# foobaz/pngloss

Hardware: AMD Instinct MI355X
Metric: Mpixels/s (filter+quantise path), 4096x4096 RGBA8 s=19; bit-exact vs ref (higher is better)
Workload: dtype u8

## Files before the change

### pngloss_amd/csrc/pl_seg_core.h

```cpp
#ifndef PL_SEG_CORE_H
#define PL_SEG_CORE_H

#include <stdint.h>
#include <stddef.h>
#include <string.h>

#include "pl_result.h"

#if defined(__HIPCC__)
#define PLS_HD __host__ __device__ __forceinline__
#else
#define PLS_HD inline
#endif

#if defined(__HIP_DEVICE_COMPILE__)
#define PLS_THREADS(tid, nt) for (int tid = (int)threadIdx.x, pls_once_ = 1; pls_once_ && tid < (int)(nt); pls_once_ = 0)
#define PLS_SYNC() __syncthreads()
#define PLS_ATOMIC_ADD(p, v) atomicAdd((p), (v))
#define PLS_ATOMIC_MIN(p, v) atomicMin((p), (v))
#define PLS_ATOMIC_OR(p, v) atomicOr((p), (v))
#define PLS_ATOMIC_CAS(p, cmp, v) atomicCAS((p), (cmp), (v))
#define PLS_ATOMIC_ADD_RET(p, v) atomicAdd((p), (v))
#define PLS_ATOMIC_EXCH(p, v) atomicExch((p), (v))
#define PLS_ATOMIC_ADD64(p, v) atomicAdd((unsigned long long *)(p), (unsigned long long)(v))
#define PLS_CLOCK() wall_clock64()
#define PLS_ATOMIC_MAX(p, v) atomicMax((p), (v))
#define PLS_WAVE_LEADER(tid) (((tid) & 63) == 0)
__device__ __forceinline__ uint32_t pls_wave_sum_u32(uint32_t v) { for (int o = 32; o > 0; o >>= 1) v += __shfl_xor(v, o, 64); return v; }
__device__ __forceinline__ uint64_t pls_wave_sum_u64(uint64_t v) { for (int o = 32; o > 0; o >>= 1) v += __shfl_xor(v, o, 64); return v; }
__device__ __forceinline__ int pls_wave_max_i(int v) { for (int o = 32; o > 0; o >>= 1) { const int t = __shfl_xor(v, o, 64); v = t > v ? t : v; } return v; }
__device__ __forceinline__ int pls_wave_min_i(int v) { for (int o = 32; o > 0; o >>= 1) { const int t = __shfl_xor(v, o, 64); v = t < v ? t : v; } return v; }
#define PLS_ATOMIC_MAX_I(p, v) atomicMax((p), (v))
#define PLS_ATOMIC_MAX_U(p, v) atomicMax((p), (v))
#define PLS_ATOMIC_MIN_I(p, v) atomicMin((p), (v))
#define PLS_HOST_VISIBLE_ADD(p, v) __hip_atomic_fetch_add((p), (v), __ATOMIC_RELAXED, __HIP_MEMORY_SCOPE_SYSTEM)
#define PLS_HOST_VISIBLE_STORE(p, v) __hip_atomic_store((p), (v), __ATOMIC_RELAXED, __HIP_MEMORY_SCOPE_SYSTEM)
#else
#define PLS_THREADS(tid, nt) for (int tid = 0; tid < (int)(nt); ++tid)
#define PLS_SYNC() ((void)0)
#define PLS_ATOMIC_ADD(p, v) (*(p) += (v))
#define PLS_ATOMIC_MIN(p, v) (*(p) = *(p) < (v) ? *(p) : (v))
#define PLS_ATOMIC_OR(p, v) (*(p) |= (v))
inline uint32_t pls_host_cas(uint32_t *p, uint32_t cmp, uint32_t v) { const uint32_t old = *p; if (old == cmp) *p = v; return old; }
inline uint32_t pls_host_add_ret(uint32_t *p, uint32_t v) { const uint32_t old = *p; *p += v; return old; }
#define PLS_ATOMIC_CAS(p, cmp, v) pls_host_cas((p), (cmp), (v))
#define PLS_ATOMIC_ADD_RET(p, v) pls_host_add_ret((p), (v))
#define PLS_ATOMIC_EXCH(p, v) (*(p) = (v))
#define PLS_ATOMIC_ADD64(p, v) (*(p) += (v))
#define PLS_CLOCK() 0ull
#define PLS_ATOMIC_MAX(p, v) (*(p) = *(p) > (v) ? *(p) : (v))
#define PLS_WAVE_LEADER(tid) (true)
inline uint32_t pls_wave_sum_u32(uint32_t v) { return v; }
inline uint64_t pls_wave_sum_u64(uint64_t v) { return v; }
inline int pls_wave_max_i(int v) { return v; }
inline int pls_wave_min_i(int v) { return v; }
#define PLS_ATOMIC_MAX_I(p, v) (*(p) = *(p) > (v) ? *(p) : (v))
#define PLS_ATOMIC_MAX_U(p, v) (*(p) = *(p) > (v) ? *(p) : (v))
#define PLS_ATOMIC_MIN_I(p, v) (*(p) = *(p) < (v) ? *(p) : (v))
#define PLS_HOST_VISIBLE_ADD(p, v) (*(p) += (v))
#define PLS_HOST_VISIBLE_STORE(p, v) (*(p) = (v))
#endif

#if defined(__HIP_DEVICE_COMPILE__) && !defined(SEG_PLAIN_POINTERS)
#define SEG_AS_LDS __attribute__((address_space(3)))
#define SEG_AS_GLB __attribute__((address_space(1)))
#else
#define SEG_AS_LDS
#define SEG_AS_GLB
#endif
typedef SEG_AS_LDS uint32_t *seg_lds_u32;
typedef SEG_AS_LDS uint8_t *seg_lds_u8;
typedef SEG_AS_LDS uint16_t *seg_lds_u16;

#if defined(__HIPCC__)
#define PLS_UNROLL _Pragma("unroll")
#else
#define PLS_UNROLL
#endif
#define SEG_NFILT 5
#ifndef SEG_DEBUG_ROW
#define SEG_DEBUG_ROW(kind, failed, winner, start_none)
#endif
#ifndef SEG_DEBUG_REPAIR
#define SEG_DEBUG_REPAIR(f, c, sg, est, sid)
#endif
#ifndef SEG_DEBUG_BREAK
#define SEG_DEBUG_BREAK(f, c, sg, est, y)
#endif
#ifndef SEG_DEBUG_STATE
#define SEG_DEBUG_STATE(f, k, sl, i, ps)
#endif
#ifndef SEG_DEBUG_COUNT
#define SEG_DEBUG_COUNT(slot, v)
#endif
#ifndef SEG_L
#define SEG_L 32
#endif
#ifndef SEG_UNIT
#define SEG_UNIT 3
#endif
#define SEG_UNIT_MIN_SEGS 680
#define SEG_SEEDS1_MIN_SEGS 330
#define SEG_SEEDS1_MIN_SEGS_PER_IMAGE 32
#define SEG_UNIT_MIN_SEGS_SEEDS 1000
#if !defined(SEG_UNC) && SEG_UNIT > 6
#define SEG_UNC 7
#endif
#ifndef SEG_UNC
#define SEG_UNC 10
#endif
#ifndef SEG_UNC_SEEDS
#define SEG_UNC_SEEDS 16
#endif
#ifndef SEG_UNC_SEEDS1
#define SEG_UNC_SEEDS1 8
#endif
#define SEG_UNC_SEEDS_OF(unit) ((unit) == 1 ? SEG_UNC_SEEDS1 : SEG_UNC_SEEDS)
#ifndef SEG_UNT
#define SEG_UNT 512
#endif
#define SEG_UPOOL SEG_UNT
#define SEG_GRP 16
#define SEG_VGRP 8
#define SEG_VGRP_UNITS 16
#ifndef SEG_TPARTS_BATCH
#define SEG_TPARTS_BATCH 1
#endif
#define SEG_VGRP_OF(tparts) ((tparts) == SEG_TPARTS_BATCH ? SEG_VGRP_UNITS : SEG_VGRP)
#define SEG_TPARTS 4
#define SEG_COMMIT_W 256
#define SEG_CTL_IMG_OF(P) (SEG_NFILT * (P).tparts)
#define SEG_PARTS 4
#define SEG_PL (SEG_L / SEG_PARTS)
#define SEG_NSP 256
#define SEG_NS_MAX 1024
#define SEG_TOFF 384
#define SEG_TN 768
#define SEG_TBL_WORDS (4 * SEG_TN + 128)
#define SEG_INVALID 0xFFFFu
#define SEG_NOFAIL 0xFFFFFFFFu
#define SEG_MAGIC 0x5E6C0DE1u
#define SEG_MAX_RESTARTS 12
#define SEG_NG_BURST 16
#define SEG_MAX_WIDTH (1u << 20)
#define SEG_THREADS 1024
#define SEG_CHAIN_THREADS 1024
#define SEG_CHAIN_THREADS_UNIT 256
#define SEG_REPLAY_THREADS (SEG_GRP * SEG_L)
#define SEG_REPLAY_NT_BATCH SEG_REPLAY_THREADS
#define SEG_REPLAY_NT (2 * SEG_REPLAY_THREADS)
#define SEG_KEYLUT_MAX 8192
#define SEG_NSS 32
#define SEG_SMALL_SEGS 8
#define SEG_ENUM_NT_SMALL_MAX_NSEG 320
#define SEG_KEYS_MAX 2048
#ifndef SEG_KA_SEEDED
#define SEG_KA_SEEDED 4
#endif
#define SEG_KIN 32
#define SEG_SEED_LANES 64
#define SEG_SEED_LONG_AFTER 2u
#define SEG_SEED_KMAX 16
#define SEG_EH 512
#define SEG_EHW 8
#define SEG_EH_WORDS (SEG_EH + SEG_EHW - 4)
#define SEG_EH_EMPTY 0xFFFFFFFFu

enum { SEG_K_INIT = 0, SEG_K_RESTART, SEG_K_RETRY, SEG_K_COMMIT, SEG_K_ABORT, SEG_K_FINISHED };

struct SegParams {
    int32_t strength, bleed;
    int32_t ns;
    int32_t dmax, cmax, tmax;
// ... 866 lines not shown
            }
            keys[tid] = key;
        }
        PLS_SYNC();
        PLS_THREADS(tid, NT) {
            if ((uint32_t)tid < DA0 + DA1) {
                const int c = (uint32_t)tid < DA0 ? 0 : 1;
                const uint32_t i = c ? (uint32_t)tid - DA0 : (uint32_t)tid;
                const uint32_t key = keys[tid];
                if (key != SEG_NOKEY && (i == 0 || keys[tid - 1] != key)) {
                    const uint32_t base = seg_eh_base(key);
                    for (int q = 0; q < SEG_EHW; q++) {
                        const uint32_t old = PLS_ATOMIC_CAS(&ht[c * SEG_EH_WORDS + base + q], SEG_NOKEY, key);
                        if (old == SEG_NOKEY) {
                            const uint32_t d = PLS_ATOMIC_ADD_RET(&trflag[SEG_TF_NDISTINCT + c], 1u);
                            dense[c * SEG_EH_WORDS + base + q] = (uint16_t)(d < SEG_NSP ? d : 0xffffu);
                            if (d < SEG_NSP) uniq[c * SEG_NSP + d] = key;
                            break;
                        }
                        if (old == key) break;
                    }
                }
            }
        }
        PLS_SYNC();
    } else {
    PLS_THREADS(tid, NT) {
        const int c = tid / SEG_NSP, i = tid % SEG_NSP;
        const uint32_t key = keys[tid];
        if (key != SEG_NOKEY && (i == 0 || keys[tid - 1] != key)) {
            const uint32_t base = seg_eh_base(key);
            for (int q = 0; q < SEG_EHW; q++) {
                const uint32_t old = PLS_ATOMIC_CAS(&ht[c * SEG_EH_WORDS + base + q], SEG_NOKEY, key);
                if (old == SEG_NOKEY) {
                    const uint32_t d = PLS_ATOMIC_ADD_RET(&trflag[SEG_TF_NDISTINCT + c], 1u);
                    dense[c * SEG_EH_WORDS + base + q] = (uint16_t)(d < SEG_NSP ? d : 0xffffu);
                    if (d < SEG_NSP) uniq[c * SEG_NSP + d] = key;
                    break;
                }
                if (old == key) break;
            }
        }
    }
    PLS_SYNC();
    }
    if (prof) te[2] = PLS_CLOCK();
    PLS_THREADS(tid, NT) {
        for (int i = tid; i < NCH * SEG_EH_WORDS; i += NT) {
            const int lc = i / SEG_EH_WORDS;
            if ((uint32_t)(c0 + lc) >= bpp) continue;
            const uint32_t k = ht[i], d = dense[i];
            j.ehash[(((size_t)f * j.nseg + seg) * 4 + c0) * SEG_EH_WORDS + i] = (k == SEG_NOKEY || d >= SEG_NSP) ? SEG_EH_EMPTY : ((k << 8) | d);
        }
    }
    PLS_THREADS(tid, NT) {
        uint32_t Dc[NCH];
        for (int k = 0; k < NCH; k++) Dc[k] = trflag[SEG_TF_NDISTINCT + k] < SEG_NSP ? trflag[SEG_TF_NDISTINCT + k] : SEG_NSP;
        int lc = 0, i = tid;
        uint32_t D = Dc[0];
        PLS_UNROLL
        for (int k = 0; k + 1 < NCH; k++) if (lc == k && (uint32_t)i >= Dc[k]) { i -= (int)Dc[k]; lc = k + 1; D = Dc[k + 1]; }
        const int c = c0 + lc;
        if (tid < NCH && (uint32_t)(c0 + tid) < bpp) j.dcnt[((size_t)f * j.nseg + seg) * 4 + c0 + tid] = trflag[SEG_TF_NDISTINCT + tid] < SEG_NSP ? trflag[SEG_TF_NDISTINCT + tid] : SEG_NSP;
        if ((uint32_t)c < bpp && (uint32_t)i < D) {
            SegState st = seg_eh_state(uniq[lc * SEG_NSP + i]);
            const size_t slot = (((size_t)f * j.nseg + seg) * 4 + c) * SEG_NSP + i;
            const SegPix *ps = px + (nrun + 1) * 4 + c;
            int bad = 0;
            for (int part = 0; part < SEG_PARTS; part++) {
                if (part) j.rck[slot * (SEG_PARTS - 1) + (part - 1)] = bad ? 0xFFFFFFFFu : seg_state_pack(st);
                bad |= seg_run_fast_f(f, trx, ps + part * SEG_PL * 4, 4, SEG_PL, st, SEG_LDS_CU32(tw), G, SEG_LDS_CU32(lut));
            }
            j.rst[slot] = bad ? 0xFFFFFFFFu : seg_state_pack(st);
        }
        if (prof && tid == 0) {
            te[3] = PLS_CLOCK(); te[4] = te[3];
            for (int q = 0; q < PLR_SEG_ENUM_PHASES; q++) { PLS_ATOMIC_MAX(&j.result[PLR_SEG_ENUM_MAX + q], (int32_t)(te[q + 1] - te[q])); PLS_ATOMIC_ADD((uint32_t *)&j.result[PLR_SEG_ENUM_SUM + q], (uint32_t)(te[q + 1] - te[q])); }
            PLS_ATOMIC_ADD((uint32_t *)&j.result[PLR_SEG_ENUM_RUNS], 1u);
            PLS_ATOMIC_ADD((uint32_t *)&j.result[PLR_SEG_ENUM_STATES], two_stage ? 2u * (trflag[SEG_TF_NDISTINCT] + trflag[SEG_TF_NDISTINCT + 1]) : trflag[SEG_TF_NDISTINCT] + trflag[SEG_TF_NDISTINCT + 1] + trflag[SEG_TF_NDISTINCT + 2] + trflag[SEG_TF_NDISTINCT + 3]);
        }
    }
}

template <int NT>
PLS_HD void seg_enum_small_body(const SegJob &j, const SegParams &P, const SegCtlView &cv, int par, int f, int seg0, unsigned char *smem)
{
    if (cv.finished || cv.active != 1) return;
    const uint32_t W = j.W, bpp = j.bpp;
    constexpr int NSEGS = NT / (4 * SEG_NSS);
    if ((uint32_t)(seg0 + NSEGS) * SEG_L <= cv.start_x) return;
    typedef SegLdsSmall<NT> LDS;
    uint32_t *tw = LDS::tw(smem), *lut = LDS::lut(smem);
    SegPix *px = LDS::px(smem);
    const uint32_t y = cv.y;
    const uint32_t *row = seg_row_orig(j, y), *nab = y ? j.img + (size_t)(y - 1u) * W : nullptr, *e0g = seg_e0(j, y);
    const SegGeo G = seg_geo((int)cv.s);
    uint32_t *trflag = LDS::trflag(smem);
    PLS_THREADS(tid, NT) { if (tid == 0) *trflag = 0u; }
    PLS_SYNC();
    PLS_THREADS(tid, NT) {
        constexpr int NTW = (SEG_TBL_WORDS + NT - 1) / NT;
        uint32_t vt[NTW], vl = 0;
        SegPixRaw vp = seg_pix_raw_zero();
        PLS_UNROLL
        for (int q = 0; q < NTW; q++) { const int i = tid + q * NT; vt[q] = i < SEG_TBL_WORDS ? j.tables[(size_t)f * SEG_TBL_WORDS + i] : 0u; }
        if (tid < 512) vl = P.lut_a[tid];
        if (tid < NSEGS * SEG_L) vp = seg_pix_fetch(row, nab, e0g, (uint32_t)seg0 * SEG_L + (uint32_t)tid, W);
        PLS_UNROLL
        for (int q = 0; q < NTW; q++) { const int i = tid + q * NT; if (i < SEG_TBL_WORDS) tw[i] = vt[q]; }
        if (tid < 512) lut[tid] = vl;
        if (tid < NSEGS * SEG_L) {
            seg_pix_split4(px + tid * 4, vp, bpp, (uint32_t)seg0 * SEG_L + (uint32_t)tid, W);
            if ((bpp & 1u) == 0u && (px[tid * 4 + (bpp - 1u)].w >> 24)) PLS_ATOMIC_OR(trflag, 1u);
        }
    }
    PLS_SYNC();
    const bool trx = *trflag != 0u;
    PLS_THREADS(tid, NT) {
        const int sl = tid / (4 * SEG_NSS), c = (tid / SEG_NSS) & 3, i = tid % SEG_NSS;
        const uint32_t seg = (uint32_t)seg0 + (uint32_t)sl, x0 = seg * SEG_L;
        if (seg < j.nseg && x0 < W && (x0 > cv.start_x || cv.start_x == 0) && (uint32_t)c < bpp && i < P.ns_small) {
            SegState st;
            uint32_t out = SEG_INVALID;
            const size_t slot = (((size_t)f * j.nseg + seg) * 4 + c) * SEG_NSP + i;
            if (seg_small_decode(P, i, st)) {
                int bad = 0;
                for (int part = 0; part < SEG_PARTS; part++) {
                    if (part) j.rck[slot * (SEG_PARTS - 1) + (part - 1)] = bad ? 0xFFFFFFFFu : seg_state_pack(st);
                    bad |= seg_run_fast_f<SEG_PL>(f, trx, px + (sl * SEG_L + part * SEG_PL) * 4 + c, 4, st, SEG_LDS_CU32(tw), G, SEG_LDS_CU32(lut));
                }
                if (!bad) out = seg_small_encode(P, st);
            } else {
                for (int part = 1; part < SEG_PARTS; part++) j.rck[slot * (SEG_PARTS - 1) + (part - 1)] = 0xFFFFFFFFu;
            }
            j.maps[(((size_t)f * j.nseg + seg) * 4 + c) * (size_t)P.nsp + i] = (uint16_t)i;
            j.rout[(((size_t)f * j.nseg + seg) * 4 + c) * SEG_NSP + i] = (uint16_t)out;
            j.rst[(((size_t)f * j.nseg + seg) * 4 + c) * SEG_NSP + i] = out == SEG_INVALID ? 0xFFFFFFFFu : seg_state_pack(st);
            if (i == 0) j.dcnt[((size_t)f * j.nseg + seg) * 4 + c] = (uint32_t)P.ns_small;
        }
    }
}

PLS_HD uint32_t seg_bits_count(const uint32_t *bits, uint32_t a, uint32_t b)
{
    uint32_t n = 0;
    for (uint32_t w = a >> 5; w <= (b ? (b - 1u) >> 5 : 0u) && a < b; w++) {
        uint32_t m = bits[w];
        if (w == (a >> 5)) m &= 0xFFFFFFFFu << (a & 31u);
        if (w == ((b - 1u) >> 5) && (b & 31u)) m &= 0xFFFFFFFFu >> (32u - (b & 31u));
        n += (uint32_t)__builtin_popcount(m);
    }
    return n;
}
template <int LANES, int UNIT, int NC, bool SEEDS = false>
PLS_HD void seg_enum_unit_body(const SegJob &j, const SegParams &P, const SegCtlView &cv, int par, int f, int grp, unsigned char *smem)
{
    if (cv.finished || cv.active != 1) return;
    constexpr int NT = SEG_UNT, HT = 2 * LANES;
    constexpr int CPR = NT / LANES < NC ? NT / LANES : NC;
    constexpr int ROUNDS = (NC + CPR - 1) / CPR;
    constexpr uint32_t E = UNIT, UL = E * SEG_L, NPX = UL + 1;
    static_assert(CPR * HT <= 2 * SEG_UNT && CPR * LANES <= SEG_UNT && NC <= 24 && NC * (UNIT * SEG_L + 1) <= SEG_UNPX, "hash tables, per-turn lists, pixel records and the bookkeeping words are sized for this");
    const uint32_t W = j.W, bpp = j.bpp, nseg = j.nseg, nunit = (nseg + E - 1) / E, ncombo = nunit * bpp;
    const uint32_t q0 = (uint32_t)grp * NC;
    if (q0 >= ncombo) return;
    const uint32_t sx = cv.start_x;
    { const uint32_t ql = seg_umin(q0 + NC, ncombo) - 1u; if (sx && (ql / bpp) * UL <= sx) return; }
    constexpr uint32_t NP1 = SEEDS ? SEG_SEED_KMAX + 1 : SEG_UN_K1MAX + 1;
    typedef SegLdsUnit<LANES, UNIT, NC, SEEDS> LDS;
    uint32_t *tw = LDS::tw(smem), *lut = LDS::lut(smem), *pool = LDS::pool(smem), *misc = LDS::misc(smem);
    uint32_t *ht = LDS::ht(smem), *uniqr = LDS::uniqr(smem), *keys = LDS::keys(smem);
    uint16_t *dense = LDS::dense(smem), *mapl = LDS::mapl(smem);
    SegPix *px1 = SEEDS ? LDS::px1_seeds(smem) : LDS::px1_std(smem);
    static_assert(!SEEDS || LANES == SEG_SEED_LANES, "one lane per seed");
    const int KR = SEEDS ? seg_min(seg_max(j.nbreak >= SEG_SEED_LONG_AFTER ? P.seed_kin + P.seed_kin / 2 : P.seed_kin, 1), SEG_SEED_KMAX) : 0;
    SegPix *px = LDS::px(smem);
    uint32_t *pool2 = LDS::pool2(smem);
    static_assert(SEG_K1 <= SEG_UN_K1MAX && SEG_K1_ONE_CHUNK <= SEG_UN_K1MAX, "the first phase's records");
    const uint32_t y = cv.y;
    const SEG_AS_GLB uint32_t *row = seg_row_orig(j, y), *nab = y ? j.img + (size_t)(y - 1u) * W : nullptr, *e0g = seg_e0(j, y);
    const SegGeo G = seg_geo((int)cv.s);
    const int nstates = seg_is_small(P, f) ? P.ns_small : P.ns;
    const bool prof = (P.engine_flags & 1) != 0 && LANES == SEG_NSP;
    unsigned long long te[5] = { 0, 0, 0, 0, 0 };
    if (prof) te[0] = PLS_CLOCK();
    PLS_THREADS(tid, NT) { if (tid < 128) misc[tid] = 0u; }
    PLS_SYNC();
    PLS_THREADS(tid, NT) {
        constexpr int NTW = (SEG_TBL_WORDS + NT - 1) / NT;
        static_assert(NC * (SEG_UN_K1MAX + 1) <= NT, "one first-phase record per thread");
        uint32_t vt[NTW], vl = 0;
        SegPix vp = seg_pix_make(0, 0, 0, 0, 0);
        PLS_UNROLL
        for (int q = 0; q < NTW; q++) { const int i = tid + q * NT; vt[q] = i < SEG_TBL_WORDS ? j.tables[(size_t)f * SEG_TBL_WORDS + i] : 0u; }
        if (tid < 512) vl = P.lut_a[tid];
        {
            const uint32_t k = (uint32_t)tid / NP1, pq = (uint32_t)tid % NP1, cq = q0 + k;
            if (k < (uint32_t)NC && cq < ncombo) {
                const uint32_t u = cq / bpp, c = cq % bpp, x = SEEDS ? u * UL + pq - 1u - (uint32_t)KR : u * UL + pq - 1u;
                if (x < W && (!SEEDS || pq <= (uint32_t)KR)) vp = seg_pix_load(row, nab, e0g, bpp, x, (int)c);
            }
        }
        PLS_UNROLL
        for (int q = 0; q < NTW; q++) { const int i = tid + q * NT; if (i < SEG_TBL_WORDS) tw[i] = vt[q]; }
        if (tid < 512) lut[tid] = vl;
        if ((uint32_t)tid < (uint32_t)NC * NP1) { px1[tid] = vp; if (vp.w >> 24) PLS_ATOMIC_OR(&misc[SEG_UM_TRANSPARENT], 1u); }
    }
    PLS_SYNC();
    const bool trx1 = misc[SEG_UM_TRANSPARENT] != 0u;
    if (prof) te[1] = PLS_CLOCK();
    const int K1 = SEEDS ? 0 : seg_k1(nstates);
    for (int r = 0; r < ROUNDS; r++) {
        PLS_THREADS(tid, NT) {
            for (int i = tid; i < CPR * HT; i += NT) ht[i] = 0xffffffffu;
            if (tid < CPR) misc[SEG_UM_TURN_N + tid] = 0u;
            if (SEEDS) for (int i = tid; i < CPR * 128; i += NT) ((uint32_t *)mapl)[i] = 0xffffffffu;
        }
        PLS_SYNC();
        if (SEEDS) {
            PLS_THREADS(tid, NT) {
                const int kk = tid / LANES, k = r * CPR + kk, i = tid % LANES;
// ... 1935 lines not shown
```

### pngloss_amd/csrc/pl_seg_lds.h

```cpp
#ifndef PL_SEG_LDS_H
#define PL_SEG_LDS_H

#ifndef PL_SEG_CORE_H
#error "pl_seg_lds.h is a part of pl_seg_core.h: include that"
#endif

#define SEG_HT 512
#ifndef SEG_UNC_SMALL
#define SEG_UNC_SMALL (SEG_UNIT <= 3 ? 20 : (SEG_UNIT <= 4 ? 15 : (SEG_UNIT <= 6 ? 10 : 7)))
#endif
#define SEG_UNC_SMALL_OF(unit) ((unit) == SEG_UNIT ? SEG_UNC_SMALL : (SEG_UNC_SMALL < 20 ? SEG_UNC_SMALL : 20))
#define SEG_UNPX (SEG_UNC_SMALL * (SEG_UNIT * SEG_L + 1))
#define SEG_UN_K1MAX 4
#define SEG_CBLK 16
#define SEG_CR_SH 6
#define SEG_CR_MAX (1 << SEG_CR_SH)
#define SEG_CHAIN_CAP 256
#define SEG_CHAIN_CAP8 224
#define SEG_CHAIN_POS (SEG_CHAIN_CAP + 32)
#define SEG_CHAIN_TROWS(n) (((n) < SEG_CHAIN_CAP8 ? (n) : SEG_CHAIN_CAP8) + SEG_CBLK + 2)
#define SEG_CHAIN_TBYTES(n) ((size_t)SEG_CHAIN_TROWS(n) * 512)
#define SEG_CHAIN_GWORDS ((SEG_CHAIN_CAP / SEG_CBLK + 2) * 256 / 2)
#ifndef SEG_WATCH_OF
#define SEG_WATCH_OF(V) ((V) > 8 ? 2 : 8)
// ... 44 lines not shown
    int first, last;
    const char *when;
};
struct SegLdsPlaced { uint32_t off[SEG_LDS_MAX_ROWS], bytes[SEG_LDS_MAX_ROWS], end; bool sound; };
constexpr SegLdsPlaced seg_lds_place(const SegLdsRegion *t, int n)
{
    SegLdsPlaced p = {};
    uint32_t rel[SEG_LDS_MAX_ROWS] = {};
    int first[SEG_LDS_MAX_ROWS] = {}, last[SEG_LDS_MAX_ROWS] = {};
    for (int k = 0; k < n; k++) {
        first[k] = t[k].kind == 2 ? first[k - 1] : t[k].first; last[k] = t[k].kind == 2 ? last[k - 1] : t[k].last;
        p.bytes[k] = t[k].count == SEG_LDS_FITS ? 0u : t[k].elem_bytes * t[k].count;
        rel[k] = t[k].kind == 2 ? rel[k - 1] + p.bytes[k - 1] : 0u;
    }
    for (int k = 0; k < n; k++)
        if (t[k].count == SEG_LDS_FITS)
            for (int q = 0; q < n; q++) if (t[q].kind && first[q] == k && last[q] == k && rel[q] + p.bytes[q] > p.bytes[k]) p.bytes[k] = rel[q] + p.bytes[q];
    for (int k = 0; k < n; k++) if (!t[k].kind) { p.off[k] = p.end; p.end += p.bytes[k]; }
    p.sound = n <= SEG_LDS_MAX_ROWS;
    for (int k = 0; k < n; k++) {
        if (t[k].kind) { p.off[k] = p.off[first[k]] + rel[k]; if (p.off[k] + p.bytes[k] > p.off[last[k]] + p.bytes[last[k]]) p.sound = false; }
        if (p.off[k] % t[k].align) p.sound = false;
    }
    return p;
}
constexpr uint32_t seg_lds_max(uint32_t a) { return a; }
template <class... R> constexpr uint32_t seg_lds_max(uint32_t a, R... r) { return a > seg_lds_max(r...) ? a : seg_lds_max(r...); }

#define SEG_LDS_ID_R(name, T, AS, n) i_##name,
#define SEG_LDS_ID_O(name, T, AS, n, first, last, when) i_##name,
#define SEG_LDS_ROW_R(name, T, AS, n) SegLdsRegion{ #name, 0u, (uint32_t)sizeof(T), (uint32_t)(n), (uint32_t)sizeof(T), 0, -1, -1, nullptr },
#define SEG_LDS_ROW_O(name, T, AS, n, first, last, when) SegLdsRegion{ #name, 0u, (uint32_t)sizeof(T), (uint32_t)(n), (uint32_t)sizeof(T), 1, i_##first, i_##last, when },
#define SEG_LDS_ROW_B(name, T, AS, n) SegLdsRegion{ #name, 0u, (uint32_t)sizeof(T), (uint32_t)(n), (uint32_t)sizeof(T), 2, -1, -1, nullptr },
#define SEG_LDS_GET_R(name, T, AS, n) static PLS_HD AS T *name(unsigned char *smem) { constexpr uint32_t o = Table::placed(0).off[Table::i_##name]; return (AS T *)((AS unsigned char *)smem + o); }
#define SEG_LDS_GET_O(name, T, AS, n, first, last, when) SEG_LDS_GET_R(name, T, AS, n)
#define SEG_LDS_VAR_BYTES(n) ((uint32_t)SEG_CHAIN_TBYTES(n))
#define SEG_LDS_GET_V(name, T, AS, n) static PLS_HD AS T *name(unsigned char *smem, uint32_t npos) { \
        constexpr uint32_t o = Table::placed(0).off[Table::i_##name] - SEG_LDS_VAR_BYTES(0); \
        static_assert(o + SEG_LDS_VAR_BYTES(60) == Table::placed(60).off[Table::i_##name] && o + SEG_LDS_VAR_BYTES(SEG_CHAIN_CAP + 1) == Table::placed(SEG_CHAIN_CAP + 1).off[Table::i_##name], "the table's offset"); \
        return (AS T *)((AS unsigned char *)smem + o + SEG_LDS_VAR_BYTES(npos)); }
#define SEG_LDS_ALIGN_X(name, bytes) if (i == i_##name) t.align = (bytes);
#define SEG_LDS_UNPAREN(...) __VA_ARGS__
#define SEG_LDS_LAYOUT(Name, LIST, ALIGN, HEAD, ARGS) \
    SEG_LDS_UNPAREN HEAD struct Name##Table { \
        enum { LIST(SEG_LDS_ID_R, SEG_LDS_ID_O, SEG_LDS_ID_R, SEG_LDS_ID_R) n_regions }; \
        static constexpr SegLdsRegion row(int i, uint32_t n) { (void)n; const SegLdsRegion all[] = { LIST(SEG_LDS_ROW_R, SEG_LDS_ROW_O, SEG_LDS_ROW_B, SEG_LDS_ROW_R) }; SegLdsRegion t = all[i]; ALIGN(SEG_LDS_ALIGN_X) return t; } \
        static constexpr SegLdsPlaced placed(uint32_t n) { SegLdsRegion t[n_regions] = {}; for (int i = 0; i < n_regions; i++) t[i] = row(i, n); return seg_lds_place(t, n_regions); } \
        static constexpr SegLdsRegion region(int i, uint32_t n = 0) { SegLdsRegion r = row(i, n); const SegLdsPlaced p = placed(n); r.offset = p.off[i]; if (r.count == SEG_LDS_FITS) r.count = p.bytes[i] / r.elem_bytes; return r; } \
        static constexpr uint32_t end(uint32_t n = 0) { return placed(n).end; } \
    }; \
    SEG_LDS_UNPAREN HEAD struct Name { \
        typedef Name##Table SEG_LDS_UNPAREN ARGS Table; \
        static_assert(Table::placed(1).sound && Table::placed(SEG_CHAIN_CAP + 1).sound, #Name ": every region starts on a multiple of its alignment, every overlay lies inside its place"); \
        LIST(SEG_LDS_GET_R, SEG_LDS_GET_O, SEG_LDS_GET_R, SEG_LDS_GET_V) \
    };

#define SEG_LDS_ALIGN_NONE(X)


#define SEG_LDS_ENUM(R, O, B, V) \
    R(tw, uint32_t, , SEG_TBL_WORDS)                   \
    R(px, SegPix, , (SEG_L + 1) * 4)                   \
    R(lut, uint32_t, , 512)                            \
    R(trflag, uint32_t, , 8)                           \
    R(ht, uint32_t, , 4 * SEG_HT)                      \
    R(dense, uint16_t, , 4 * SEG_HT)                   \
    R(uniq, uint32_t, , 4 * SEG_NSP)                   \
    R(res, uint16_t, , 4 * SEG_NSP)                    \
    R(lslot, uint16_t, , NT)                           \
    R(keys, uint32_t, , NT)
SEG_LDS_LAYOUT(SegLdsEnum, SEG_LDS_ENUM, SEG_LDS_ALIGN_NONE, (template <int NT>), (<NT>))

#define SEG_LDS_SEEDED(R, O, B, V) \
    R(tw, uint32_t, , SEG_TBL_WORDS) \
    R(px, SegPix, , (SEG_KIN + SEG_L + 1) * 4)         \
    R(lut, uint32_t, , 512) \
    R(trflag, uint32_t, , 8)                           \
    R(ht, uint32_t, , 4 * SEG_EH_WORDS)                \
    R(dense, uint16_t, , 4 * SEG_EH_WORDS)             \
    R(uniq, uint32_t, , 4 * SEG_NSP)                   \
    R(keys, uint32_t, , NT)
SEG_LDS_LAYOUT(SegLdsSeeded, SEG_LDS_SEEDED, SEG_LDS_ALIGN_NONE, (template <int NT>), (<NT>))

#define SEG_LDS_SMALL(R, O, B, V) \
    R(tw, uint32_t, , SEG_TBL_WORDS) \
    R(lut, uint32_t, , 512) \
    R(px, SegPix, , NT / (4 * SEG_NSS) * SEG_L * 4)    \
    R(trflag, uint32_t, , 1)
SEG_LDS_LAYOUT(SegLdsSmall, SEG_LDS_SMALL, SEG_LDS_ALIGN_NONE, (template <int NT>), (<NT>))

#define SEG_LDS_UNIT_CPR (SEG_UNT / LANES < NC ? SEG_UNT / LANES : NC)
#define SEG_LDS_UNIT(R, O, B, V) \
    R(tw, uint32_t, , SEG_TBL_WORDS) \
    R(lut, uint32_t, , 512) \
    R(pool, uint32_t, , SEG_UPOOL)                     \
    R(px1_std, SegPix, , SEG_UNC_SMALL * (SEG_UN_K1MAX + 1))    \
    R(misc, uint32_t, , 128)                           \
    R(work, unsigned char, , SEG_LDS_FITS) \
    O(ht, uint32_t, , 2 * SEG_UNT, work, work, "in the first phase")    \
    B(dense, uint16_t, , 2 * SEG_UNT)                  \
    B(uniqr, uint32_t, , SEG_UNT)                      \
    B(keys, uint32_t, , SEG_UNT)                       \
    B(px1_seeds, SegPix, , SEEDS ? NC * (SEG_SEED_KMAX + 1) : 0)    \
    B(mapl, uint16_t, , SEEDS ? SEG_LDS_UNIT_CPR * 256 : 0)      \
    O(px, SegPix, , SEG_UNPX, work, work, "in the second phase, behind the barrier that ends the first")    \
    B(pool2, uint32_t, , SEG_UPOOL)
SEG_LDS_LAYOUT(SegLdsUnit, SEG_LDS_UNIT, SEG_LDS_ALIGN_NONE, (template <int LANES, int UNIT, int NC, bool SEEDS>), (<LANES, UNIT, NC, SEEDS>))

#define SEG_LDS_FIRST(R, O, B, V) \
    R(tw, uint32_t, , SEG_TBL_WORDS) \
    R(lut, uint32_t, , 512) \
    R(Hf, uint32_t, , 256)                             \
    R(rank, uint32_t, , 256) \
    R(px, SegPix, , (UNITS ? SEG_UNIT : 1) * SEG_L * 4)
SEG_LDS_LAYOUT(SegLdsFirst, SEG_LDS_FIRST, SEG_LDS_ALIGN_NONE, (template <int NT, bool UNITS>), (<NT, UNITS>))

#define SEG_LDS_CHAIN(R, O, B, V) \
    R(Hf, uint32_t, SEG_AS_LDS, 256)                   \
    R(rank, uint32_t, SEG_AS_LDS, 256)                 \
    R(lut, uint32_t, SEG_AS_LDS, 512)                  \
    R(idxb, uint32_t, SEG_AS_LDS, 32)                  \
    R(dn, uint32_t, SEG_AS_LDS, SEG_CHAIN_POS)         \
    R(entL, uint32_t, SEG_AS_LDS, SEG_CHAIN_POS)       \
    R(G, uint16_t, SEG_AS_LDS, 2 * SEG_CHAIN_GWORDS)   \
    R(T, uint16_t, SEG_AS_LDS, SEG_CHAIN_TBYTES(n) / 2)    \
    V(twr, uint32_t, SEG_AS_LDS, SEEDED ? SEG_TBL_WORDS : 0)    \
    V(pxr, SegPix, SEG_AS_LDS, SEEDED ? SEG_L + 1 : 0)
#define SEG_LDS_CHAIN_ALIGN(X) X(T, 16)
SEG_LDS_LAYOUT(SegLdsChain, SEG_LDS_CHAIN, SEG_LDS_CHAIN_ALIGN, (template <bool SEEDED>), (<SEEDED>))

#define SEG_LDS_EXTREMES(R, O, B, V) \
    R(mm, uint32_t, , 2)
SEG_LDS_LAYOUT(SegLdsExtremes, SEG_LDS_EXTREMES, SEG_LDS_ALIGN_NONE, (), ())

#define SEG_LDS_REPLAY(R, O, B, V) \
    R(Hf, uint32_t, , 256) \
    R(rank, uint32_t, , 256) \
    R(lut, uint32_t, , 512) \
    R(tw, uint32_t, , SEG_TBL_WORDS) \
    R(px, SegPix, , SEG_GRP * SEG_L * 4)               \
    R(cnt, uint32_t, , SEG_GRP * 64)                   \
    R(lane, uint32_t, , SEG_GRP * SEG_PARTS * 4 * 2)   \
    R(cwl, uint32_t, , SEG_REPLAY_THREADS * 4)         \
    R(oaL, uint32_t, , SEG_REPLAY_THREADS + 3)         \
    O(rm, uint32_t, , 768, tw, tw, "behind the walk")   \
    B(red, uint32_t, , 16)                             \
    B(h0s, uint32_t, , 256)
#define SEG_LDS_REPLAY_ALIGN(X) X(red, 8)
SEG_LDS_LAYOUT(SegLdsReplay, SEG_LDS_REPLAY, SEG_LDS_REPLAY_ALIGN, (), ())

#define SEG_LDS_POST(R, O, B, V) \
    R(H0, uint32_t, , 256) \
    R(rank, uint32_t, , 256) \
    R(spare, uint32_t, , 256)                          \
    R(cum, uint32_t, , (VGRP + 1) * 256)               \
    R(cw, uint32_t, , (VGRP * SEG_L + 2) * 4)          \
    R(red, uint32_t, , 64)                             \
    R(lut, uint32_t, , 512)                            \
    R(ro, uint32_t, , VGRP * SEG_L + 2)                \
    R(na, uint32_t, , VGRP * SEG_L + 2)                \
    R(e0, uint32_t, , 2 * VGRP * SEG_L)                \
    R(wbits, uint32_t, , 32)                           \
    R(slot_of, uint8_t, , 256)                         \
    R(pend, uint8_t, , VGRP * SEG_L * 4)               \
    R(binb, uint8_t, , VGRP * SEG_BINB_STRIDE)         \
    R(pcw, uint32_t, , SEG_WATCH_OF(VGRP) * SEG_PC_STRIDE_V(VGRP))    \
    R(btop, uint32_t, , 2 * SEG_NBAND * 4)             \
    R(hiG, uint32_t, , 256) \
    R(loG, uint32_t, , 256) \
    O(cumx, uint32_t, , (SEG_GRP - VGRP) * 256, pcw, pcw, "while staging, before pcw is written: barriers lie between")
SEG_LDS_LAYOUT(SegLdsPost, SEG_LDS_POST, SEG_LDS_ALIGN_NONE, (template <int VGRP>), (<VGRP>))

// ... 72 lines not shown
```

Baseline: 96.45.

## Tabulate per-pixel state transitions for small-seg enumeration and walk tables per seed

In the small enumeration path, each pixel record is now evaluated once for every possible incoming cn value, and the resulting next-state (cn, th) and left bits are stored in LDS transition tables. Each seed lane then walks these tables with cheap lookups instead of rerunning the full per-pixel step function for its own state, falling back to the original loop when a state overflows the table range. This removes redundant step computation across the seeds that share the same pixels, at the cost of extra LDS space, an additional barrier and a table-build phase.

```diff
diff --git a/pngloss_amd/csrc/pl_seg_core.h b/pngloss_amd/csrc/pl_seg_core.h
--- a/pngloss_amd/csrc/pl_seg_core.h
+++ b/pngloss_amd/csrc/pl_seg_core.h
@@ -89,6 +89,9 @@
 #endif
 #ifndef SEG_DEBUG_STATE
 #define SEG_DEBUG_STATE(f, k, sl, i, ps)
+#endif
+#ifndef SEG_DEBUG_SMALL
+#define SEG_DEBUG_SMALL(tables, walked, out)
 #endif
 #ifndef SEG_DEBUG_COUNT
 #define SEG_DEBUG_COUNT(slot, v)
@@ -1121,16 +1124,57 @@
     }
 }
 
-template <int NT>
+PLS_HD uint32_t seg_small_lane_loop(const SegJob &j, const SegParams &P, int f, bool trx, const SegPix *pxl, int i, size_t slot, const uint32_t *tw, const uint32_t *lut, const SegGeo &G)
+{
+    SegState st;
+    uint32_t out = SEG_INVALID;
+    if (seg_small_decode(P, i, st)) {
+        int bad = 0;
+        for (int part = 0; part < SEG_PARTS; part++) {
+            if (part) j.rck[slot * (SEG_PARTS - 1) + (part - 1)] = bad ? 0xFFFFFFFFu : seg_state_pack(st);
+            bad |= seg_run_fast_f<SEG_PL>(f, trx, pxl + part * SEG_PL * 4, 4, st, SEG_LDS_CU32(tw), G, SEG_LDS_CU32(lut));
+        }
+        if (!bad) out = seg_small_encode(P, st);
+    } else {
+        for (int part = 1; part < SEG_PARTS; part++) j.rck[slot * (SEG_PARTS - 1) + (part - 1)] = 0xFFFFFFFFu;
+    }
+    j.rout[slot] = (uint16_t)out;
+    j.rst[slot] = out == SEG_INVALID ? 0xFFFFFFFFu : seg_state_pack(st);
+    return out;
+}
+#define SEG_SMALL_NONE 0x80FFu
+template <int F, bool TRX, int NT>
+PLS_HD void seg_small_eval(int cmax, const SegPix &rec, int q, int qb, const SegStepMem &M, const SegGeo &G, SEG_AS_LDS uint16_t *ct, SEG_AS_LDS uint8_t *bk)
+{
+#if defined(__HIPCC__)
+    _Pragma("unroll 3")
+#endif
+    for (int k = 0; k <= 2 * cmax; k++) {
+        SegState st;
+        st.left = 0; st.cn = k - cmax; st.th = 0;
+        int bad = 0;
+        seg_step_fast<F, TRX>(rec, st, bad, M, G);
+        const bool ok = !seg_bad(bad) && st.cn >= -64 && st.cn <= 64 && st.th >= -64 && st.th <= 64;
+        ct[k * NT + q] = (uint16_t)(ok ? (uint32_t)(st.cn + 128) | (uint32_t)(st.th + 128) << 8 : SEG_SMALL_NONE);
+        if (qb >= 0) bk[k * (NT / SEG_PL) + qb] = (uint8_t)st.left;
+    }
+}
+template <int NT, bool TABLES = true>
 PLS_HD void seg_enum_small_body(const SegJob &j, const SegParams &P, const SegCtlView &cv, int par, int f, int seg0, unsigned char *smem)
 {
     if (cv.finished || cv.active != 1) return;
     const uint32_t W = j.W, bpp = j.bpp;
     constexpr int NSEGS = NT / (4 * SEG_NSS);
+    static_assert(NSEGS * SEG_L * 4 == NT, "the table path: one pixel record per thread");
     if ((uint32_t)(seg0 + NSEGS) * SEG_L <= cv.start_x) return;
     typedef SegLdsSmall<NT> LDS;
     uint32_t *tw = LDS::tw(smem), *lut = LDS::lut(smem);
     SegPix *px = LDS::px(smem);
+    const int ns = P.ns_small, cmax = P.cmax, tmax = P.tmax;
+    const bool tab = TABLES && seg_small_tables_fit<NT>(ns, cmax, tmax);
+    SEG_AS_LDS uint32_t *sts = LDS::sts(smem);
+    SEG_AS_LDS uint16_t *ct = LDS::ct(smem);
+    SEG_AS_LDS uint8_t *kl = LDS::kl(smem), *bk = LDS::bk(smem);
     const uint32_t y = cv.y;
     const uint32_t *row = seg_row_orig(j, y), *nab = y ? j.img + (size_t)(y - 1u) * W : nullptr, *e0g = seg_e0(j, y);
     const SegGeo G = seg_geo((int)cv.s);
@@ -1139,12 +1183,17 @@
     PLS_SYNC();
     PLS_THREADS(tid, NT) {
         constexpr int NTW = (SEG_TBL_WORDS + NT - 1) / NT;
-        uint32_t vt[NTW], vl = 0;
+        static_assert(SEG_SMALL_KL <= NT && SEG_NSS <= NT, "one entry of the set's tables per thread");
+        uint32_t vt[NTW], vl = 0, vs = 0;
+        uint16_t vk = (uint16_t)SEG_INVALID;
         SegPixRaw vp = seg_pix_raw_zero();
+        const int kn = tab ? (2 * cmax + 1) * (2 * tmax + 1) : 0;
         PLS_UNROLL
         for (int q = 0; q < NTW; q++) { const int i = tid + q * NT; vt[q] = i < SEG_TBL_WORDS ? j.tables[(size_t)f * SEG_TBL_WORDS + i] : 0u; }
         if (tid < 512) vl = P.lut_a[tid];
         if (tid < NSEGS * SEG_L) vp = seg_pix_fetch(row, nab, e0g, (uint32_t)seg0 * SEG_L + (uint32_t)tid, W);
+        if (tid < kn) vk = P.keylut_small[tid];
+        if (tab && tid < SEG_NSS) vs = P.st_small[tid];
         PLS_UNROLL
         for (int q = 0; q < NTW; q++) { const int i = tid + q * NT; if (i < SEG_TBL_WORDS) tw[i] = vt[q]; }
         if (tid < 512) lut[tid] = vl;
@@ -1152,30 +1201,63 @@
             seg_pix_split4(px + tid * 4, vp, bpp, (uint32_t)seg0 * SEG_L + (uint32_t)tid, W);
             if ((bpp & 1u) == 0u && (px[tid * 4 + (bpp - 1u)].w >> 24)) PLS_ATOMIC_OR(trflag, 1u);
         }
+        if (tid < kn) kl[tid] = (uint8_t)(vk == (uint16_t)SEG_INVALID ? 255u : vk);
+        if (tab && tid < SEG_NSS) sts[tid] = vs;
     }
     PLS_SYNC();
     const bool trx = *trflag != 0u;
+    if (tab) {
+        PLS_THREADS(tid, NT) {
+            const int sl = tid / (SEG_L * 4), pl = (tid >> 2) & (SEG_L - 1), c = tid & 3;
+            const uint32_t seg = (uint32_t)seg0 + (uint32_t)sl, x0 = seg * SEG_L;
+            if (seg < j.nseg && x0 < W && (x0 > cv.start_x || cv.start_x == 0) && (uint32_t)c < bpp) {
+                const SegPix rec = px[tid];
+                const SegStepMem M = seg_step_mem(SEG_LDS_CU32(tw), SEG_LDS_CU32(lut));
+                const int qb = (pl % SEG_PL) == SEG_PL - 1 ? (sl * SEG_PARTS + pl / SEG_PL) * 4 + c : -1;
+                if (f == 2) { if (trx) seg_small_eval<2, true, NT>(cmax, rec, tid, qb, M, G, ct, bk); else seg_small_eval<2, false, NT>(cmax, rec, tid, qb, M, G, ct, bk); }
+                else { if (trx) seg_small_eval<0, true, NT>(cmax, rec, tid, qb, M, G, ct, bk); else seg_small_eval<0, false, NT>(cmax, rec, tid, qb, M, G, ct, bk); }
+            }
+        }
+        PLS_SYNC();
+    }
     PLS_THREADS(tid, NT) {
         const int sl = tid / (4 * SEG_NSS), c = (tid / SEG_NSS) & 3, i = tid % SEG_NSS;
         const uint32_t seg = (uint32_t)seg0 + (uint32_t)sl, x0 = seg * SEG_L;
-        if (seg < j.nseg && x0 < W && (x0 > cv.start_x || cv.start_x == 0) && (uint32_t)c < bpp && i < P.ns_small) {
-            SegState st;
-            uint32_t out = SEG_INVALID;
+        if (seg < j.nseg && x0 < W && (x0 > cv.start_x || cv.start_x == 0) && (uint32_t)c < bpp && i < ns) {
             const size_t slot = (((size_t)f * j.nseg + seg) * 4 + c) * SEG_NSP + i;
-            if (seg_small_decode(P, i, st)) {
-                int bad = 0;
+            bool walked = false;
+            if (tab) {
+                SEG_AS_LDS const uint16_t *ctl = ct + sl * (SEG_L * 4) + c;
+                SEG_AS_LDS const uint8_t *bkl = bk + sl * SEG_PARTS * 4 + c;
+                const uint32_t w0 = sts[i], top = 2u * (uint32_t)cmax;
+                uint32_t ci = (w0 & 255u) - 128u + (uint32_t)cmax, tb = ((w0 >> 8) & 255u) - 256u + (uint32_t)cmax, over = 0, ck[SEG_PARTS];
+                PLS_UNROLL
                 for (int part = 0; part < SEG_PARTS; part++) {
-                    if (part) j.rck[slot * (SEG_PARTS - 1) + (part - 1)] = bad ? 0xFFFFFFFFu : seg_state_pack(st);
-                    bad |= seg_run_fast_f<SEG_PL>(f, trx, px + (sl * SEG_L + part * SEG_PL) * 4 + c, 4, st, SEG_LDS_CU32(tw), G, SEG_LDS_CU32(lut));
-                }
-                if (!bad) out = seg_small_encode(P, st);
-            } else {
-                for (int part = 1; part < SEG_PARTS; part++) j.rck[slot * (SEG_PARTS - 1) + (part - 1)] = 0xFFFFFFFFu;
-            }
+                    uint32_t from = ci;
+                    PLS_UNROLL
+                    for (int q = 0; q < SEG_PL; q++) {
+                        from = ci;
+                        const uint32_t e = ctl[from * NT + (uint32_t)(part * SEG_PL + q) * 4];
+                        const uint32_t nc = (e & 255u) + tb;
+                        tb = (e >> 8) - 256u + (uint32_t)cmax;
+                        over |= nc > top ? 1u : 0u; ci = seg_umin(nc, top);
+                    }
+                    ck[part] = (uint32_t)bkl[from * (NT / SEG_PL) + (uint32_t)part * 4] | ((ci - (uint32_t)cmax + 32768u) & 0xffffu) << 8 | ((tb - (uint32_t)cmax + 256u) & 255u) << 24;
+                }
+                if (!over) {
+                    walked = true;
+                    const uint32_t ti = tb - (uint32_t)cmax + 128u + (uint32_t)tmax;
+                    const uint32_t out = ti <= 2u * (uint32_t)tmax && kl[ci * (2u * (uint32_t)tmax + 1u) + ti] != 255u ? (uint32_t)kl[ci * (2u * (uint32_t)tmax + 1u) + ti] : (uint32_t)SEG_INVALID;
+                    PLS_UNROLL
+                    for (int part = 1; part < SEG_PARTS; part++) j.rck[slot * (SEG_PARTS - 1) + (part - 1)] = ck[part - 1];
+                    j.rout[slot] = (uint16_t)out;
+                    j.rst[slot] = out == SEG_INVALID ? 0xFFFFFFFFu : ck[SEG_PARTS - 1];
+                }
+            }
+            if (!walked) { const uint32_t out = seg_small_lane_loop(j, P, f, trx, px + (sl * SEG_L) * 4 + c, i, slot, tw, lut, G); (void)out; SEG_DEBUG_SMALL(tab, false, out); }
+            else SEG_DEBUG_SMALL(tab, true, 0u);
             j.maps[(((size_t)f * j.nseg + seg) * 4 + c) * (size_t)P.nsp + i] = (uint16_t)i;
-            j.rout[(((size_t)f * j.nseg + seg) * 4 + c) * SEG_NSP + i] = (uint16_t)out;
-            j.rst[(((size_t)f * j.nseg + seg) * 4 + c) * SEG_NSP + i] = out == SEG_INVALID ? 0xFFFFFFFFu : seg_state_pack(st);
-            if (i == 0) j.dcnt[((size_t)f * j.nseg + seg) * 4 + c] = (uint32_t)P.ns_small;
+            if (i == 0) j.dcnt[((size_t)f * j.nseg + seg) * 4 + c] = (uint32_t)ns;
         }
     }
 }
diff --git a/pngloss_amd/csrc/pl_seg_lds.h b/pngloss_amd/csrc/pl_seg_lds.h
--- a/pngloss_amd/csrc/pl_seg_lds.h
+++ b/pngloss_amd/csrc/pl_seg_lds.h
@@ -150,12 +150,25 @@
     R(keys, uint32_t, , NT)
 SEG_LDS_LAYOUT(SegLdsSeeded, SEG_LDS_SEEDED, SEG_LDS_ALIGN_NONE, (template <int NT>), (<NT>))
 
+#define SEG_SMALL_KL 256
+#define SEG_SMALL_ROOM(NT) (SegLdsEnum<NT>::Table::end() - (uint32_t)(SEG_TBL_WORDS * 4 + 512 * 4 + (NT) / (4 * SEG_NSS) * SEG_L * 4 * sizeof(SegPix) + 4 + SEG_NSS * 4 + SEG_SMALL_KL))
+#define SEG_SMALL_NCN(NT) (SEG_SMALL_ROOM(NT) / (2u * (NT) + (NT) / SEG_PL))
 #define SEG_LDS_SMALL(R, O, B, V) \
     R(tw, uint32_t, , SEG_TBL_WORDS) \
     R(lut, uint32_t, , 512) \
     R(px, SegPix, , NT / (4 * SEG_NSS) * SEG_L * 4)    \
-    R(trflag, uint32_t, , 1)
+    R(trflag, uint32_t, , 1)                           \
+    R(sts, uint32_t, SEG_AS_LDS, SEG_NSS)              \
+    R(ct, uint16_t, SEG_AS_LDS, SEG_SMALL_NCN(NT) * NT)    \
+    R(kl, uint8_t, SEG_AS_LDS, SEG_SMALL_KL)           \
+    R(bk, uint8_t, SEG_AS_LDS, SEG_SMALL_ROOM(NT) - 2u * SEG_SMALL_NCN(NT) * NT)
 SEG_LDS_LAYOUT(SegLdsSmall, SEG_LDS_SMALL, SEG_LDS_ALIGN_NONE, (template <int NT>), (<NT>))
+static_assert(SegLdsSmall<512>::Table::end() == SegLdsEnum<512>::Table::end() && SegLdsSmall<1024>::Table::end() == SegLdsEnum<1024>::Table::end(), "the tables of none / up fill what seg_enum_body's layout leaves them, no more");
+static_assert(SEG_SMALL_ROOM(512) - 2u * SEG_SMALL_NCN(512) * 512 >= SEG_SMALL_NCN(512) * (512 / SEG_PL) && SEG_SMALL_ROOM(1024) - 2u * SEG_SMALL_NCN(1024) * 1024 >= SEG_SMALL_NCN(1024) * (1024 / SEG_PL), "bk holds a byte per value of cn and part");
+template <int NT> constexpr bool seg_small_tables_fit(int ns, int cmax, int tmax)
+{
+    return ns > 0 && ns <= SEG_NSS && cmax >= 0 && tmax >= 0 && cmax <= 30 && tmax <= 30 && (uint32_t)(2 * cmax + 1) <= SEG_SMALL_NCN(NT) && (2 * cmax + 1) * (2 * tmax + 1) <= SEG_SMALL_KL;
+}
 
 #define SEG_LDS_UNIT_CPR (SEG_UNT / LANES < NC ? SEG_UNT / LANES : NC)
 #define SEG_LDS_UNIT(R, O, B, V) \
```

New measurement: 99.28 (median of 6 runs). 2.9% higher.
